# bonlime/sota_imagenet

Measured on AMD Instinct MI355X. Metric: images/sec (whole node) ResNet-50 bs=256/GPU @224px, higher is better.
Workload: dtype bf16; 1 GPU; ResNet-50 v1.5 train step (fwd+CE+bwd+allreduce+SGD), bs=256/GPU, 224px, configs[2] bf16 activations / fp32 accumulate+master; global_batch=256, image_size=224, parallelism=dp1

## Files before the change

### include/mi355rn.h

```cpp
#ifndef MI355RN_H
#define MI355RN_H

#include <stddef.h>
#include <stdint.h>

#ifdef __cplusplus
extern "C" {
#endif

typedef enum mi355_status {
  MI355_OK = 0,
  MI355_E_ARG = -1,
  MI355_E_HIP = -2,
  MI355_E_STATE = -3,
  MI355_E_NOMEM = -4
} mi355_status;

typedef enum mi355_dtype { MI355_F32 = 0, MI355_BF16 = 1, MI355_FP8 = 2 } mi355_dtype;

const char* mi355_last_error(void);
int mi355_version(void);
int mi355_device_count(void);


// ... 52 lines not shown
int mi355_stem_ingest(int dtype, const float* x_nchw, void* xpad, int N, int H, int W, void* stream);
int mi355_stem_fwd(int dtype, const void* xpad, const float* w_krsc, void* y, int N, int H, int W,
                   void* ws, size_t ws_bytes, void* stream);
int mi355_stem_wgrad(int dtype, const void* dy, const void* xpad, float* dw, float beta, int N, int H,
                     int W, void* ws, size_t ws_bytes, void* stream);
size_t mi355_stem_workspace_bytes(int dtype, int N, int H, int W);

size_t mi355_bn_workspace_bytes(int C);
int mi355_bn_fwd_train(int dtype, const void* x, const void* residual, void* out, const float* gamma,
                       const float* beta, float* running_mean, float* running_var, float* save_mean,
                       float* save_invstd, int M, int C, float eps, float momentum, int relu, void* ws,
                       size_t ws_bytes, void* stream);
int mi355_bn_fwd_train_partial(int dtype, const void* x, const void* residual, void* out, const float* gamma,
                               const float* beta, float* running_mean, float* running_var, float* save_mean,
                               float* save_invstd, int M, int C, float eps, float momentum, int relu, const float* partial,
                               int nblk, void* ws, size_t ws_bytes, void* stream);
int mi355_bn_fwd_eval(int dtype, const void* x, const void* residual, void* out, const float* gamma,
                      const float* beta, const float* running_mean, const float* running_var, int M,
                      int C, float eps, int relu, void* ws, size_t ws_bytes, void* stream);
int mi355_bn_bwd(int dtype, const void* dout, const void* out, const void* x, const float* gamma,
                 const float* save_mean, const float* save_invstd, void* dx, void* dz_out,
                 float* dgamma, float* dbeta, float beta_acc, int M, int C, int relu, void* ws,
                 size_t ws_bytes, void* stream);

int mi355_maxpool_fwd(int dtype, const void* x, void* y, uint8_t* idx, int N, int H, int W, int C,
                      void* stream);
int mi355_maxpool_bwd(int dtype, const void* dy, const uint8_t* idx, void* dx, int N, int H, int W,
                      int C, void* stream);

int mi355_gap_fwd(int dtype, const void* x, float* pooled, int N, int HW, int C, void* stream);
int mi355_gap_bwd(int dtype, const float* dpooled, void* dx, int N, int HW, int C, void* stream);

int mi355_ce_loss(const float* logits, const float* target, float smoothing, float grad_scale,
                  float* loss, float* row_loss, float* dlogits, int N, int C, void* stream);

int mi355_sgd_step(float* p, const float* g, float* m, size_t n, float lr, float momentum,
                   float weight_decay, float grad_scale, void* stream);
int mi355_sgd_step_ema(float* p, const float* g, float* m, float* ema, size_t n, float lr, float momentum,
                       float weight_decay, float grad_scale, float ema_decay, void* stream);

int mi355_adam_step(float* p, const float* g, float* m, float* v, size_t n, double beta1, double beta2, float eps,
                    float step_size, float bc2_sqrt, double lr, double weight_decay, int decoupled, float grad_scale,
                    void* stream);
int mi355_adam_step_ema(float* p, const float* g, float* m, float* v, float* ema, size_t n, double beta1, double beta2,
                        float eps, float step_size, float bc2_sqrt, double lr, double weight_decay, int decoupled,
                        float grad_scale, float ema_decay, void* stream);
// ... 164 lines not shown
```

### sota_imagenet_amd/csrc/bn.hip

```cpp
#include <hip/hip_fp8.h>

#include <algorithm>

#include "common.h"
#include "vec.h"

namespace mi355 {
namespace {

constexpr int MAXBLK = 512;

__device__ __forceinline__ void quant8(const float (&v)[8], float scale, uint8_t* dst, float& amax) {
  float c[8];
#pragma unroll
  for (int e = 0; e < 8; ++e) {
    const float r = (float)(bf16_t)v[e];
    amax = fmaxf(amax, fabsf(r));
    c[e] = __builtin_amdgcn_fmed3f(r * scale, 448.f, -448.f);
  }
  int lo = 0, hi = 0;
  lo = __builtin_amdgcn_cvt_pk_fp8_f32(c[0], c[1], lo, false);
  lo = __builtin_amdgcn_cvt_pk_fp8_f32(c[2], c[3], lo, true);
  hi = __builtin_amdgcn_cvt_pk_fp8_f32(c[4], c[5], hi, false);
  hi = __builtin_amdgcn_cvt_pk_fp8_f32(c[6], c[7], hi, true);
// ... 6 lines not shown
  if ((threadIdx.x & 63) == 0) wmax[threadIdx.x >> 6] = amax;
  __syncthreads();
  if (threadIdx.x == 0) {
    const float m = fmaxf(fmaxf(wmax[0], wmax[1]), fmaxf(wmax[2], wmax[3]));
    if (m > __uint_as_float(__atomic_load_n(dst, __ATOMIC_RELAXED))) atomicMax(dst, __float_as_uint(m));
  }
}

template <int V>
__device__ __forceinline__ void load_consts(const float* __restrict__ p, int c0, float (&v)[V]) {
#pragma unroll
  for (int q = 0; q < V / 4; ++q) {
    const f32x4 t = *reinterpret_cast<const f32x4*>(p + c0 + 4 * q);
    v[4 * q] = t[0]; v[4 * q + 1] = t[1]; v[4 * q + 2] = t[2]; v[4 * q + 3] = t[3];
  }
}

template <typename T, int V>
__device__ __forceinline__ void eca_grad(const EcaGrad& eg, int n, int C, int c0, float (&gv)[V]) {
  const float kn = eg.keep ? eg.keep[n] : 1.f;
  const size_t o = (size_t)n * C + c0;
#pragma unroll
  for (int e = 0; e < V; ++e) gv[e] = (float)(T)(gv[e] * kn * eg.gate[o + e] + eg.dpool[o + e]);
}

struct ReduceArgs {
  const void* x;
  const void* g;
  const void* mask;
  const uint8_t* bits;
  void* dz_out;
  const float* mean;
  const float* invstd;
  float* partial;
  float* pivot;
  int M, C;
  float slope;
  EcaGrad eg;
};

template <typename T, int MODE, int MASK, bool DZ>
__global__ __launch_bounds__(256) void bn_reduce_kernel(const ReduceArgs p) {
  constexpr int V = Vec16<T>::N;
  __shared__ __attribute__((aligned(16))) float red[2][256 * V];
  const int tpr_full = p.C / V;
  const int tpr = tpr_full < 256 ? tpr_full : 256;
// ... 47 lines not shown
#pragma unroll
        for (int e = 0; e < V; ++e) gv[e] = (b >> e) & 1u ? gv[e] : 0.f;
      } else if constexpr (MASK == 3) {
        const unsigned b = p.bits[off / V];
#pragma unroll
        for (int e = 0; e < V; ++e) gv[e] = (b >> e) & 1u ? gv[e] : gv[e] * p.slope;
      } else if constexpr (MASK == 1) {
        float mv[V];
        Vec16<T>::load(mk + off, mv);
#pragma unroll
        for (int e = 0; e < V; ++e) gv[e] = mv[e] > 0.f ? gv[e] : gv[e] * p.slope;
      } else if constexpr (MASK == 4) {
        eca_grad<T, V>(p.eg, m / p.eg.hw, p.C, c0, gv);
      }
      if constexpr (DZ) Vec16<T>::store(dz_out + off, gv);
#pragma unroll
      for (int e = 0; e < V; ++e) {
        const float xh = (xv[e] - mu[e]) * is[e];
        s1[e] += gv[e];
        s2[e] += gv[e] * xh;
      }
    }
  }
  int nrows, myrow;
  bool writer;
  if (tpr < 64) {
    for (int off = tpr; off < 64; off <<= 1) {
#pragma unroll
      for (int e = 0; e < V; ++e) {
        s1[e] += __shfl_xor(s1[e], off);
        s2[e] += __shfl_xor(s2[e], off);
      }
    }
    nrows = 4;
    myrow = tid >> 6;
    writer = (tid & 63) < tpr;
  } else {
    nrows = rpp;
    myrow = r;
    writer = true;
  }
  if (writer) {
#pragma unroll
    for (int e = 0; e < V; ++e) {
      red[0][(myrow * tpr + cv) * V + e] = s1[e];
      red[1][(myrow * tpr + cv) * V + e] = s2[e];
    }
  }
  __syncthreads();
  if (tid < tpr) {
#pragma unroll
    for (int e = 0; e < V; ++e) {
      float a = 0.f, b = 0.f;
      for (int rr = 0; rr < nrows; ++rr) {
        a += red[0][(rr * tpr + tid) * V + e];
        b += red[1][(rr * tpr + tid) * V + e];
      }
      const int c = (blockIdx.y * tpr + tid) * V + e;
      p.partial[((size_t)blockIdx.x * 2 + 0) * p.C + c] = a;
      p.partial[((size_t)blockIdx.x * 2 + 1) * p.C + c] = b;
    }
  }
}

struct FinalizeArgs {
  const float* partial;
  const float* pivot;
  int nblk, M, C;
  const float* gamma;
  const float* beta;
  float* running_mean;
  float* running_var;
  float* save_mean;
  float* save_invstd;
  float* scale;
  float* shift;
  float eps, momentum;
  const float* invstd;
  float* dgamma;
  float* dbeta;
  float beta_acc;
  float* coef;
};

static int fin_wide_mode() { return 2; }
// ... 151 lines not shown
#pragma unroll
      for (int e = 0; e < V; ++e) v[e] = v[e] > 0.f ? v[e] : (RELU == 2 ? 0.f : v[e] * p.slope);
    }
    if constexpr (!QONLY) Vec16<T>::store(out + i * V, v);
    if constexpr (Q) quant8(v, qs, p.qo.q + i * V, amax);
  }
  if constexpr (Q) amax_flush(amax, p.qo.amax);
}

struct BwdApplyArgs {
  const void* g;
  const void* mask;
  const uint8_t* bits;
  const void* x;
  const float* mean;
  const float* invstd;
  const float* coef;
  void* dx;
  size_t nvec;
  int cvecs, C;
  float slope;
  EcaGrad eg;
  QuantOut qo;
};

template <typename T, int MASK, bool Q = false, bool QONLY = false>
__global__ __launch_bounds__(256) void bn_bwd_apply_kernel(const BwdApplyArgs p) {
  constexpr int V = Vec16<T>::N;
  static_assert(!Q || V == 8, "the quantised twin exists for bf16 tensors");
  float qs = 1.f, amax = 0.f;
  if constexpr (Q) qs = p.qo.scale[0];
  const T* g = reinterpret_cast<const T*>(p.g);
  const T* mk = reinterpret_cast<const T*>(p.mask);
  const T* x = reinterpret_cast<const T*>(p.x);
  T* dx = reinterpret_cast<T*>(p.dx);
  const size_t stride = (size_t)gridDim.x * 256;
  size_t i = (size_t)blockIdx.x * 256 + threadIdx.x;
  const int c0 = (int)(i % p.cvecs) * V;
  float mu[V], is[V], k0[V], k1[V], k2[V];
  load_consts<V>(p.mean, c0, mu);
  load_consts<V>(p.invstd, c0, is);
  load_consts<V>(p.coef, c0, k0);
  load_consts<V>(p.coef + p.C, c0, k1);
  load_consts<V>(p.coef + 2 * p.C, c0, k2);
#pragma unroll 2
  for (; i < p.nvec; i += stride) {
    float gv[V], xv[V];
    Vec16<T>::load_nt(g + i * V, gv);
    Vec16<T>::load_nt(x + i * V, xv);
    if constexpr (MASK == 2) {
      const unsigned b = p.bits[i];
#pragma unroll
      for (int e = 0; e < V; ++e) gv[e] = (b >> e) & 1u ? gv[e] : 0.f;
    } else if constexpr (MASK == 3) {
      const unsigned b = p.bits[i];
#pragma unroll
      for (int e = 0; e < V; ++e) gv[e] = (b >> e) & 1u ? gv[e] : gv[e] * p.slope;
    } else if constexpr (MASK == 4) {
      eca_grad<T, V>(p.eg, (int)((i / p.cvecs) / (size_t)p.eg.hw), p.C, c0, gv);
    } else if constexpr (MASK == 1) {
      float mv[V];
      Vec16<T>::load(mk + i * V, mv);
#pragma unroll
      for (int e = 0; e < V; ++e) gv[e] = mv[e] > 0.f ? gv[e] : gv[e] * p.slope;
    }
#pragma unroll
    for (int e = 0; e < V; ++e) {
      const float xh = (xv[e] - mu[e]) * is[e];
      gv[e] = k0[e] * (gv[e] - k1[e] - xh * k2[e]);
    }
    if constexpr (!QONLY) Vec16<T>::store(dx + i * V, gv);
    if constexpr (Q) quant8(gv, qs, p.qo.q + i * V, amax);
  }
  if constexpr (Q) amax_flush(amax, p.qo.amax);
}

constexpr int SC = 64;

__device__ __forceinline__ __amdgpu_buffer_rsrc_t rsrc_of(const void* p, size_t bytes) {
  return __builtin_amdgcn_make_buffer_rsrc(const_cast<void*>(p), 0, (int)(bytes > 0xfffffffcull ? 0xfffffffcull : bytes), 0x00020000);
}
__device__ __forceinline__ uint4 buf16(__amdgpu_buffer_rsrc_t r, unsigned voff, unsigned soff, bool nt = false) {
  return nt ? __builtin_bit_cast(uint4, __builtin_amdgcn_raw_buffer_load_b128(r, voff, soff, 2))
            : __builtin_bit_cast(uint4, __builtin_amdgcn_raw_buffer_load_b128(r, voff, soff, 0));
}

template <typename T>
struct PoolGather {
  static constexpr int V = Vec16<T>::N;
  uint4 g[4];
  uint32_t id[4][V / 4];
  __device__ __forceinline__ void load(__amdgpu_buffer_rsrc_t rg, __amdgpu_buffer_rsrc_t ri, unsigned t, unsigned cv, int a, int b, int Ho, int Wo) {
    const unsigned go = (t * SC + cv * V) * (unsigned)sizeof(T), io = t * SC + cv * V;
#pragma unroll
    for (int w = 0; w < 4; ++w) {
      const bool ok = a + (w >> 1) < Ho && b + (w & 1) < Wo;
      const unsigned srow = (w >> 1) ? (unsigned)Wo * SC : 0u;
// ... 396 lines not shown

int launch_bn_bwd_finalize(const float* partial, int nblk, int M, int C, const float* gamma, const float* invstd,
                           float* dgamma, float* dbeta, float beta_acc, float* coef, hipStream_t s) {
  FinalizeArgs a{};
  a.partial = partial;
  a.nblk = nblk;
  a.M = M;
  a.C = C;
  a.gamma = gamma;
  a.invstd = invstd;
  a.dgamma = dgamma;
  a.dbeta = dbeta;
  a.beta_acc = beta_acc;
  a.coef = coef;
  if (fin_one_channel(C, nblk) && nblk > FIN_WIDE_ROWS) hipLaunchKernelGGL((bn_finalize_kernel<1, 1, 1024>), dim3(C), dim3(1024), 0, s, a);
  else if (fin_one_channel(C, nblk)) hipLaunchKernelGGL((bn_finalize_kernel<1, 1>), dim3(C), dim3(256), 0, s, a);
  else hipLaunchKernelGGL((bn_finalize_kernel<1, 4>), dim3(C / 4), dim3(256), 0, s, a);
  MI355_LAUNCH_CHECK();
  return 0;
}

int launch_bn_bwd_apply(int dtype, const void* g, const void* mask_src, const void* x, const float* mean,
                        const float* invstd, const float* coef, void* dx, int M, int C, hipStream_t s,
                        const uint8_t* relu_bits, float slope, QuantOut qo, const EcaGrad* eg) {
  MI355_TRY(check_c(dtype, C));
  const int V = 16 / (int)dtype_size(dtype);
  BwdApplyArgs a{};
  if (eg) a.eg = *eg;
  a.slope = slope;
  a.g = g;
  a.mask = mask_src;
  a.bits = relu_bits;
  a.x = x;
  a.mean = mean;
  a.invstd = invstd;
  a.coef = coef;
  a.dx = dx;
  a.nvec = (size_t)M * C / V;
  a.cvecs = C / V;
  a.C = C;
  const int blocks = elementwise_blocks(a.nvec, a.cvecs);
  const int mask = relu_bits ? (slope != 0.f ? 3 : 2) : mask_src ? 1 : 0;
  a.qo = qo;
  if (eg) {
    MI355_ARG(mask == 0 && !qo.q && eg->gate && eg->dpool && eg->hw > 0, "bn_bwd_apply: the ECA gradient source takes no mask / twin");
    if (dtype == MI355_F32) hipLaunchKernelGGL((bn_bwd_apply_kernel<float, 4>), dim3(blocks), dim3(256), 0, s, a);
    else hipLaunchKernelGGL((bn_bwd_apply_kernel<bf16_t, 4>), dim3(blocks), dim3(256), 0, s, a);
    MI355_LAUNCH_CHECK();
    return 0;
  }
  if (qo.q) {
    MI355_ARG(dtype == MI355_BF16 && mask != 1 && mask != 3 && qo.scale && qo.amax, "bn_bwd_apply: the e4m3 twin needs bf16 and a ReLU bit mask (or none)");
    if (mask == 2 && qo.only) hipLaunchKernelGGL((bn_bwd_apply_kernel<bf16_t, 2, true, true>), dim3(blocks), dim3(256), 0, s, a);
    else if (mask == 2) hipLaunchKernelGGL((bn_bwd_apply_kernel<bf16_t, 2, true>), dim3(blocks), dim3(256), 0, s, a);
    else if (qo.only) hipLaunchKernelGGL((bn_bwd_apply_kernel<bf16_t, 0, true, true>), dim3(blocks), dim3(256), 0, s, a);
    else hipLaunchKernelGGL((bn_bwd_apply_kernel<bf16_t, 0, true>), dim3(blocks), dim3(256), 0, s, a);
    MI355_LAUNCH_CHECK();
    return 0;
  }
#define MI355_BN_BWD_APPLY(TT)                                                                                  \
  switch (mask) {                                                                                               \
    case 0: hipLaunchKernelGGL((bn_bwd_apply_kernel<TT, 0>), dim3(blocks), dim3(256), 0, s, a); break;          \
    case 1: hipLaunchKernelGGL((bn_bwd_apply_kernel<TT, 1>), dim3(blocks), dim3(256), 0, s, a); break;          \
    case 2: hipLaunchKernelGGL((bn_bwd_apply_kernel<TT, 2>), dim3(blocks), dim3(256), 0, s, a); break;          \
    default: hipLaunchKernelGGL((bn_bwd_apply_kernel<TT, 3>), dim3(blocks), dim3(256), 0, s, a); break;         \
  }
// ... 55 lines not shown
```

### sota_imagenet_amd/csrc/common.h

```cpp
#pragma once
#include <hip/hip_runtime.h>
#include <cstdarg>
#include <cstdint>
#include <cstdio>
#include <cstring>

#include "../../include/mi355rn.h"

namespace mi355 {

typedef __bf16 bf16_t;

typedef float f32x4 __attribute__((ext_vector_type(4)));
typedef float f32x16 __attribute__((ext_vector_type(16)));
typedef __bf16 bf16x8 __attribute__((ext_vector_type(8)));
typedef __bf16 bf16x4 __attribute__((ext_vector_type(4)));
typedef short s16x4 __attribute__((ext_vector_type(4)));

void set_error(const char* fmt, ...);
int device_cus();
int probe_env(const char* name);

#define MI355_HIP(expr)                                                                         \
  do {                                                                                          \
// ... 181 lines not shown
                       float* scale, float* shift, float eps, float momentum, hipStream_t s);
int launch_bn_eval_coeffs(const float* gamma, const float* beta, const float* rm, const float* rv, float* scale,
                          float* shift, int C, float eps, hipStream_t s);
struct QuantOut {
  uint8_t* q = nullptr;
  const float* scale = nullptr;
  unsigned* amax = nullptr;
  bool only = false;
};
int launch_bn_apply(int dtype, const void* x, const float* scale, const float* shift, const void* residual,
                    const void* x2, const float* scale2, const float* shift2, void* out, int M, int C, int relu,
                    hipStream_t s, uint8_t* relu_bits = nullptr, QuantOut qo = QuantOut());
struct EcaGrad {
  const float* keep = nullptr;
  const float* gate = nullptr;
  const float* dpool = nullptr;
  int hw = 0;
};
int launch_bn_bwd_reduce(int dtype, const void* g, const void* mask_src, const void* x, const float* mean,
                         const float* invstd, void* dz_out, float* partial, int* nblk_out, int M, int C,
                         hipStream_t s, const uint8_t* relu_bits = nullptr, float slope = 0.f, const EcaGrad* eg = nullptr);
int launch_bn_bwd_finalize(const float* partial, int nblk, int M, int C, const float* gamma, const float* invstd,
                           float* dgamma, float* dbeta, float beta_acc, float* coef , hipStream_t s);
int launch_bn_bwd_apply(int dtype, const void* g, const void* mask_src, const void* x, const float* mean,
                        const float* invstd, const float* coef, void* dx, int M, int C, hipStream_t s,
                        const uint8_t* relu_bits = nullptr, float slope = 0.f, QuantOut qo = QuantOut(), const EcaGrad* eg = nullptr);
int launch_stem_bwd_reduce(int dtype, const void* dp, const uint8_t* idx, const uint8_t* bits, const void* y, const float* mean,
                           const float* invstd, float* partial, int* nblk_out, int N, int H, int W, int C, hipStream_t s);
int launch_stem_bwd_apply(int dtype, const void* dp, const uint8_t* idx, const uint8_t* bits, const void* y, const float* mean,
                          const float* invstd, const float* coef, void* dx, int N, int H, int W, int C, hipStream_t s);
int bn_max_blocks();
int launch_nchw_pad64(int dtype, const float* x_nchw, void* h_nhwc64, int N, int HW, hipStream_t s);
int launch_weight_pad_cast(int dtype, const float* w, void* wp, int Cout, int taps, int Cin, int Coutp, int Cinp, hipStream_t s);
int launch_nchw_im2col3s2(int dtype, const float* x, void* h, int N, int H, int W, hipStream_t s);
int launch_weight_unpad(const float* dwp, float* dw, float beta, int Cout, int taps, int Cin, int Cinp, hipStream_t s);
int launch_axpby(const float* src, float* dst, float beta, size_t n, hipStream_t s);
int launch_eca_residual_fwd(int dtype, const void* x, const float* w, int k, const float* keep, const void* shortcut, void* out, float* pooled, float* gate,
                            int N, int HW, int C, int act, hipStream_t s, const float* xs = nullptr, const float* xh = nullptr, const float* ss = nullptr,
                            const float* sh2 = nullptr, uint8_t* out_bits = nullptr, float* raw_ws = nullptr );
int launch_eca_residual_bwd(int dtype, const void* dout, const void* out, const void* x, const float* keep, const float* w, int k, const float* pooled,
                            const float* gate, void* dshortcut, void* dx, float* dw, float beta, float* ws, int N, int HW, int C, int act, hipStream_t s,
                            const float* xs = nullptr, const float* xh = nullptr, float* bn_row = nullptr, const float* bn_mean = nullptr,
                            const float* bn_invstd = nullptr, const uint8_t* out_bits = nullptr, const void* ds_y = nullptr, float* ds_row = nullptr,
                            const float* ds_mean = nullptr, const float* ds_invstd = nullptr);
int launch_fp8_scale_update(float* scale, unsigned* amax, int n, float headroom, hipStream_t s);

int launch_maxpool_fwd(int dtype, const void* x, void* y, uint8_t* idx, int N, int H, int W, int C, hipStream_t s);
int launch_bn_relu_maxpool(int dtype, const void* y, const float* scale, const float* shift, void* p, uint8_t* idx,
                           uint8_t* bits, int N, int H, int W, int C, hipStream_t s);
// ... 52 lines not shown
```

### sota_imagenet_amd/csrc/conv_api.cpp

```cpp
#include <algorithm>
#include <atomic>
#include <cstdio>
#include <cstdlib>
#include <mutex>
#include <set>
#include <string>

#include "conv_kernels.h"

namespace mi355 {

static thread_local std::string g_err;

void set_error(const char* fmt, ...) {
  char buf[1024];
  va_list ap;
  va_start(ap, fmt);
  vsnprintf(buf, sizeof(buf), fmt, ap);
  va_end(ap);
  g_err = buf;
}
const char* get_error() { return g_err.c_str(); }

int probe_env(const char* name) {
// ... 452 lines not shown
  MI355_ARG(ws && ws_bytes >= (size_t)2 * C * 4, "bn_eval: workspace too small");
  hipStream_t s = (hipStream_t)stream;
  float* scale = (float*)ws;
  float* shift = scale + C;
  MI355_TRY(launch_bn_eval_coeffs(gamma, beta, running_mean, running_var, scale, shift, C, eps, s));
  return launch_bn_apply(dtype, x, scale, shift, residual, nullptr, nullptr, nullptr, out, M, C, relu, s);
}

int mi355_bn_bwd(int dtype, const void* dout, const void* out, const void* x, const float* gamma,
                 const float* save_mean, const float* save_invstd, void* dx, void* dz_out, float* dgamma,
                 float* dbeta, float beta_acc, int M, int C, int relu, void* ws, size_t ws_bytes, void* stream) {
  MI355_ARG(ws && ws_bytes >= mi355_bn_workspace_bytes(C), "bn: workspace too small");
  hipStream_t s = (hipStream_t)stream;
  float* partial = (float*)ws;
  float* coef = partial + (size_t)bn_max_blocks() * 2 * C;
  int nblk = 0;
  const void* mask = relu ? out : nullptr;
  const float slope = relu == 2 ? 0.01f : 0.f;
  MI355_TRY(launch_bn_bwd_reduce(dtype, dout, mask, x, save_mean, save_invstd, dz_out, partial, &nblk, M, C, s, nullptr, slope));
  MI355_TRY(launch_bn_bwd_finalize(partial, nblk, M, C, gamma, save_invstd, dgamma, dbeta, beta_acc, coef, s));
  return launch_bn_bwd_apply(dtype, dout, mask, x, save_mean, save_invstd, coef, dx, M, C, s, nullptr, slope);
}

int mi355_maxpool_fwd(int dtype, const void* x, void* y, uint8_t* idx, int N, int H, int W, int C, void* stream) {
  return launch_maxpool_fwd(dtype, x, y, idx, N, H, W, C, (hipStream_t)stream);
}
int mi355_maxpool_bwd(int dtype, const void* dy, const uint8_t* idx, void* dx, int N, int H, int W, int C,
                      void* stream) {
  return launch_maxpool_bwd(dtype, dy, idx, dx, N, H, W, C, (hipStream_t)stream);
}
int mi355_gap_fwd(int dtype, const void* x, float* pooled, int N, int HW, int C, void* stream) {
  return launch_gap_fwd(dtype, x, pooled, N, HW, C, (hipStream_t)stream);
}
int mi355_gap_bwd(int dtype, const float* dpooled, void* dx, int N, int HW, int C, void* stream) {
  return launch_gap_bwd(dtype, dpooled, dx, N, HW, C, (hipStream_t)stream);
}
int mi355_ce_loss(const float* logits, const float* target, float smoothing, float grad_scale, float* loss,
                  float* row_loss, float* dlogits, int N, int C, void* stream) {
  return launch_ce(logits, target, smoothing, grad_scale, loss, row_loss, dlogits, N, C, (hipStream_t)stream);
}
int mi355_sgd_step(float* p, const float* g, float* m, size_t n, float lr, float momentum, float weight_decay,
                   float grad_scale, void* stream) {
  return launch_sgd(p, g, m, n, lr, momentum, weight_decay, grad_scale, (hipStream_t)stream);
}
int mi355_sgd_step_ema(float* p, const float* g, float* m, float* ema, size_t n, float lr, float momentum, float weight_decay,
                       float grad_scale, float ema_decay, void* stream) {
// ... 119 lines not shown
```

### sota_imagenet_amd/csrc/resnet_exec.cpp

```cpp
#include <cstdlib>
#include <string>
#include <vector>

#include "flat_model.h"

namespace mi355 {

namespace {

constexpr float BN_EPS = 1e-5f;
constexpr float FP8_HEADROOM = 2.f;
constexpr size_t PARAM_ALIGN = 64;
constexpr int MAX_EVENTS = 8192;

struct ConvBN {
  std::string conv_name, bn_name;
  int Cin, Cout, K, stride, pad;
  int Hin, Win, Hout, Wout;
  size_t w_off = 0, gamma_off = 0, beta_off = 0;
  size_t rm_off = 0, rv_off = 0;
  void* y = nullptr;
  void* w_cast = nullptr;
  void* w_tr = nullptr;
  float* stat = nullptr;
// ... 42 lines not shown
  uint8_t* a0_bits = nullptr;
  float *pooled = nullptr, *fc_tmp = nullptr, *dlogits_pad = nullptr, *dpooled = nullptr, *fc_wtr = nullptr;
  float *bn_partial = nullptr, *bn_coef = nullptr, *wg_partial = nullptr;
  float *bn_partial2 = nullptr, *bn_coef2 = nullptr;
  void* sk_ws[2] = {nullptr, nullptr};
  bool stream_k = true;
  bool fp8 = false;
  int q_n = 0;
  float* q_scale = nullptr;
  unsigned* q_amax = nullptr;
  void* gq[MAX_GSETS][4] = {};
  bool fp8_fwd_cal = false, fp8_bwd_cal = false;
  bool fp8_fwd_on = false, fp8_bwd_on = false;
  bool fp8_use_fwd = true, fp8_use_bwd = true;
  bool fp8_use_wgrad = true;
  bool fp8_keep_bf16 = false;
  bool fp8_lean = false;
  unsigned* sk_err_host = nullptr;
  PrepDesc* prep_table[2] = {nullptr, nullptr};
  int prep_layers = 0, prep_tiles = 0;
  void* gG[2] = {nullptr, nullptr};
  void* gsub = nullptr;
  bool ds_compact = true;
  void* gset[MAX_GSETS][4] = {};
  size_t max_c = 64;
  int nsets = 2;
  bool fuse_bn_bwd = false;
  bool fuse_bn_in = true;
  bool stem_fused_bwd = true;
  hipEvent_t w_done[MAX_GSETS] = {};
  hipEvent_t ds_done = nullptr;
  bool w_pending[MAX_GSETS] = {};
  int bwd_parity = 0;
  bool fwd_training_done = false;
  int next_seg = 0;
  void* cur_dout = nullptr;
  double fwd_flops = 0, train_flops = 0;

  unsigned prof_mask = 0;
  std::vector<hipEvent_t> ev;
  struct Rec {
    int cls;
    int tag;
    double flops, bytes;
  };
  std::vector<Rec> recs;
// ... 41 lines not shown
  hipStream_t stream;
  int idx = -1;
  Prof(mi355_ctx* ctx, int cls, double flops, double bytes, hipStream_t s, int tag = 0) : c(ctx), stream(s) {
    if (!(c->prof_mask & (1u << cls))) return;
    if ((c->recs.size() + 1) * 2 > c->ev.size()) return;
    idx = (int)c->recs.size();
    c->recs.push_back({cls, tag, flops, bytes});
    (void)hipEventRecord(c->ev[2 * idx], stream);
  }
  ~Prof() {
    if (idx >= 0) (void)hipEventRecord(c->ev[2 * idx + 1], stream);
  }
};

enum { PC_IGEMM128 = 0, PC_IGEMM64 = 1, PC_WGRAD128 = 2, PC_WGRAD64 = 3, PC_BN_REDUCE = 4, PC_BN_APPLY = 5, PC_OTHER = 6,
       PC_BN_BWD_APPLY = 7 };
inline int igemm_class(int ncols) { return ncols % 128 == 0 ? PC_IGEMM128 : PC_IGEMM64; }
inline int wgrad_class(int cout) { return cout % 128 == 0 ? PC_WGRAD128 : PC_WGRAD64; }

inline float* bn_partial_of(mi355_ctx* c, hipStream_t s) { return (c->wstream && s == c->wstream) ? c->bn_partial2 : c->bn_partial; }
inline void* sk_ws_of(mi355_ctx* c, hipStream_t s) {
  return c->stream_k ? c->sk_ws[(c->wstream && s == c->wstream) ? 1 : 0] : nullptr;
}
inline float* bn_coef_of(mi355_ctx* c, hipStream_t s) { return (c->wstream && s == c->wstream) ? c->bn_coef2 : c->bn_coef; }
double conv_flops(const mi355_ctx* c, const ConvBN& l) {
  return 2.0 * c->N * l.Hout * l.Wout * (double)l.Cout * l.Cin * l.K * l.K;
}

int conv_forward(mi355_ctx* c, ConvBN& l, const void* in, int training, float momentum, hipStream_t s, const ConvBN* bn_in = nullptr,
                 void* a_out = nullptr, uint8_t* a_bits = nullptr) {
  IgemmArgs a;
  build_fwd_args(a, c->N, l.Hin, l.Win, l.Cin, l.Cout, l.K, l.K, l.stride, l.pad);
  a.in = in;
  if (bn_in) {
    a.bn_in = bn_in->stat + 2 * bn_in->Cout;
    a.bn_in_a = a_out;
    a.bn_in_bits = a_bits;
  }
  a.stat_partial = training ? bn_partial_of(c, s) : nullptr;
  a.stat_rows_cap = (int)((size_t)bn_max_blocks() * c->max_c / l.Cout);
  a.sk_ws = sk_ws_of(c, s);
  a.wt = c->dtype == MI355_F32 ? (const void*)(c->params + l.w_off) : (const void*)l.w_cast;
  a.out = l.y;
  const double fl = conv_flops(c, l);
  const bool q = training && c->fp8_fwd_on && l.fp8_fwd;
  const double by = (double)c->N * l.Hin * l.Win * l.Cin * (q ? 1 : c->es) * (bn_in ? 2.0 + 1.0 / 16 : 1.0) + (double)c->N * l.Hout * l.Wout * l.Cout * c->es;
// ... 44 lines not shown

int bn_apply(mi355_ctx* c, ConvBN& l, const void* residual, ConvBN* l2, void* out, int relu, hipStream_t s,
             uint8_t* bits, uint8_t* q = nullptr, int qid = -1, bool q_only = false) {
  const int M = c->N * l.Hout * l.Wout, C = l.Cout;
  const int nin = 1 + (residual ? 1 : 0) + (l2 ? 1 : 0);
  QuantOut qo;
  if (q && bits && qid >= 0) {
    qo.q = q; qo.scale = c->q_scale + qid; qo.amax = c->q_amax + qid;
    qo.only = q_only && !residual && !l2;
  }
  Prof p(c, PC_BN_APPLY, 0, (double)M * C * (c->es * (nin + (qo.only ? 0 : 1)) + (qo.q ? 1 : 0)), s);
  return launch_bn_apply(c->dtype, l.y, l.stat + 2 * C, l.stat + 3 * C, residual, l2 ? l2->y : nullptr,
                         l2 ? l2->stat + 2 * C : nullptr, l2 ? l2->stat + 3 * C : nullptr, out, M, C, relu, s, bits, qo);
}

void* grad_twin(const mi355_ctx* c, const void* g) {
  for (int p = 0; p < c->nsets; ++p)
    for (int i = 0; i < 4; ++i)
      if (c->gset[p][i] == g) return c->gq[p][i];
  return nullptr;
}

int bn_backward(mi355_ctx* c, ConvBN& l, const void* g, const uint8_t* bits, void* dz_out, void* dx, float beta_acc,
                hipStream_t s) {
  const int M = c->N * l.Hout * l.Wout, C = l.Cout;
  int nblk = l.bwd_rows;
  l.bwd_rows = 0;
  const double mask_bytes = bits ? (double)M * C * c->es / 16 : 0.0;
  if (nblk == 0 || dz_out) {
    Prof p(c, PC_BN_REDUCE, 0, (double)M * C * c->es * (2 + (dz_out ? 1 : 0)) + mask_bytes, s);
    MI355_TRY(launch_bn_bwd_reduce(c->dtype, g, nullptr, l.y, l.stat, l.stat + C, dz_out, bn_partial_of(c, s), &nblk, M, C, s,
                                   bits, 0.f));
  }
  MI355_TRY(launch_bn_bwd_finalize(bn_partial_of(c, s), nblk, M, C, c->params + l.gamma_off, l.stat + C,
                                     c->grads + l.gamma_off, c->grads + l.beta_off, beta_acc, bn_coef_of(c, s), s));
  const uint8_t* bits2 = dz_out ? nullptr : bits;
  const void* g2 = dz_out ? dz_out : g;
  QuantOut qo;
  if (c->fp8 && l.qid_dy >= 0) {
    qo.q = (uint8_t*)grad_twin(c, dx); qo.scale = c->q_scale + l.qid_dy; qo.amax = c->q_amax + l.qid_dy;
    qo.only = c->fp8_lean && c->fp8_bwd_on && l.fp8_dgrad && l.fp8_wgrad && qo.q;
  }
  Prof p(c, PC_BN_BWD_APPLY, 0, (double)M * C * (c->es * (qo.only ? 2 : 3) + (qo.q ? 1 : 0)) + (bits2 ? mask_bytes : 0.0), s);
  return launch_bn_bwd_apply(c->dtype, g2, nullptr, l.y, l.stat, l.stat + C, bn_coef_of(c, s), dx, M, C, s, bits2, 0.f, qo);
}

int conv_wgrad(mi355_ctx* c, ConvBN& l, const void* dy, const void* x, float beta_acc, hipStream_t s) {
  WgradArgs a;
  build_wgrad_args(a, c->N, l.Hin, l.Win, l.Cin, l.Cout, l.K, l.K, l.stride, l.pad);
  a.dy = dy; a.x = x; a.partial = c->wg_partial;
  const size_t n = (size_t)l.Cout * l.K * l.K * l.Cin;
  void* dyq = c->fp8_bwd_on && l.fp8_wgrad ? grad_twin(c, dy) : nullptr;
  const double by = ((double)c->N * l.Hin * l.Win * l.Cin + (double)c->N * l.Hout * l.Wout * l.Cout) * (dyq ? 1 : c->es);
  if (dyq) {
    a.dy = dyq; a.x = l.in_q;
    {
      Prof p(c, wgrad_class(l.Cout), conv_flops(c, l), by, s, 2);
      MI355_TRY(launch_wgrad(MI355_FP8, a, l.splits8, s));
    }
    snprintf(l.k_wgrad, sizeof(l.k_wgrad), "%s", mi355_last_conv_kernel());
    return launch_splitk_reduce(c->wg_partial, l.splits8, n, c->grads + l.w_off, n, beta_acc, s, c->q_scale + l.qid_dy, c->q_scale + l.qid_in);
  }
  {
    Prof p(c, wgrad_class(l.Cout), conv_flops(c, l), by, s);
    MI355_TRY(launch_wgrad(c->dtype, a, l.splits, s));
  }
  snprintf(l.k_wgrad, sizeof(l.k_wgrad), "%s", mi355_last_conv_kernel());
// ... 238 lines not shown
  const int splits = plan_wgrad_splits(MI355_F32, N, P, 1, 2048);
  hipStream_t ws;
  MI355_TRY(c->fork(s, &ws));
  MI355_TRY(launch_wgrad(MI355_F32, w, splits, ws));
  MI355_TRY(launch_splitk_reduce(c->wg_partial, splits, (size_t)P * 2048, c->grads + c->fc_w_off, (size_t)O * 2048,
                                 beta_acc, ws));
  MI355_TRY(launch_fc(c->dlogits_pad, c->fc_wtr, c->dpooled, N, 2048, P, s));
  const Block& last = c->blocks.back();
  c->cur_dout = c->gG[0];
  c->bwd_parity = 0;
  return launch_gap_bwd(c->dtype, c->dpooled, c->cur_dout, N, last.Hout * last.Wout, last.Cout, s);
}

int backward_block(mi355_ctx* c, Block& b, Block* prev, float beta_acc, hipStream_t s) {
  void* G = c->cur_dout;
  void* Gn = G == c->gG[0] ? c->gG[1] : c->gG[0];
  const int par = c->bwd_parity;
  c->bwd_parity = (par + 1) % c->nsets;
  void** S = c->gset[par];
  void *B1 = S[0], *B2 = S[1], *B3 = S[2], *B4 = S[3];
  hipStream_t ws;
  const bool sub2 = sub2_ok(c, b, prev);
  MI355_TRY(acquire_set(c, par, s));
  MI355_TRY(bn_backward(c, b.c3, G, b.out_bits, nullptr, B1, beta_acc, s));
  MI355_TRY(c->fork(s, &ws));
  MI355_TRY(conv_wgrad(c, b.c3, B1, b.a2, beta_acc, ws));
  if (b.has_ds) {
    MI355_TRY(bn_backward(c, b.ds, G, b.out_bits, nullptr, B2, beta_acc, ws));
    if (sub2) MI355_TRY(conv_dgrad_compact(c, b.ds, B2, c->gsub, ws));
    else MI355_TRY(conv_dgrad(c, b.ds, B2, Gn, nullptr, ws));
    if (c->overlap) MI355_HIP(hipEventRecord(c->ds_done, ws));
    MI355_TRY(conv_wgrad(c, b.ds, B2, b.in, beta_acc, ws));
  }
  MI355_TRY(conv_dgrad(c, b.c3, B1, B3, nullptr, s, nullptr, &b.c2, b.a2_bits, beta_acc));
  MI355_TRY(bn_backward(c, b.c2, B3, b.a2_bits, nullptr, B3, beta_acc, s));
  MI355_TRY(c->fork(s, &ws));
  MI355_TRY(conv_wgrad(c, b.c2, B3, b.a1, beta_acc, ws));
  MI355_TRY(conv_dgrad(c, b.c2, B3, B4, nullptr, s, nullptr, &b.c1, b.a1_bits, beta_acc));
  MI355_TRY(bn_backward(c, b.c1, B4, b.a1_bits, nullptr, B4, beta_acc, s));
  MI355_TRY(c->fork(s, &ws));
  MI355_TRY(conv_wgrad(c, b.c1, B4, b.in, beta_acc, ws));
  if (b.has_ds) {
    if (c->overlap) MI355_HIP(hipStreamWaitEvent(s, c->ds_done, 0));
    MI355_TRY(conv_dgrad(c, b.c1, B4, Gn, sub2 ? c->gsub : Gn, s, nullptr, prev ? &prev->c3 : nullptr, prev ? prev->out_bits : nullptr, beta_acc, sub2));
    c->cur_dout = Gn;
  } else {
    MI355_TRY(conv_dgrad(c, b.c1, B4, G, G, s, b.out_bits, prev ? &prev->c3 : nullptr, prev ? prev->out_bits : nullptr, beta_acc));
// ... 109 lines not shown
  double f = conv_flops(c, c->stem), bw = 2 * conv_flops(c, c->stem) - conv_flops(c, c->stem);
  double tr = 2 * conv_flops(c, c->stem);
  (void)bw;
  for (auto& b : c->blocks) {
    const double fb = conv_flops(c, b.c1) + conv_flops(c, b.c2) + conv_flops(c, b.c3) + (b.has_ds ? conv_flops(c, b.ds) : 0);
    f += fb;
    tr += 3 * fb;
  }
  const double ffc = 2.0 * N * 2048 * num_classes;
  c->fwd_flops = f + ffc;
  c->train_flops = tr + 3 * ffc;

  const char* bad = nullptr;
  if (c->fp8) {
    plan_fp8(c, &bad);
    c->fp8_use_fwd = env_switch("MI355_FP8_FWD", 1, 1, &bad) != 0;
    c->fp8_use_bwd = env_switch("MI355_FP8_BWD", 1, 1, &bad) != 0;
  }
  c->stream_k = env_switch("MI355_STREAM_K", 1, 1, &bad) != 0;
  c->fuse_bn_bwd = env_switch("MI355_FUSE_BN_BWD", dtype == MI355_BF16 ? 1 : 0, 1, &bad) != 0;
  c->stem_fused_bwd = env_switch("MI355_STEM_FUSED", 1, 1, &bad) != 0;
  c->overlap = env_switch("MI355_WGRAD_STREAM", 1, 1, &bad) != 0;
  c->ds_compact = env_switch("MI355_DS_COMPACT", 1, 1, &bad) != 0;
  if (bad) {
    set_error("create: %s=%s is outside the switch's domain", bad, getenv(bad));
    mi355_resnet50_destroy(c);
    return MI355_E_ARG;
  }
  Arena ar;
  plan_arena(c, ar);
  c->arena_bytes = ar.size;
  if (device < 0) {
    *out = c;
    return 0;
  }
  hipError_t e = hipMalloc((void**)&c->arena, ar.size);
  if (e != hipSuccess) {
    set_error("create: hipMalloc(%zu bytes) -> %s", ar.size, hipGetErrorString(e));
    delete c;
    return MI355_E_NOMEM;
  }
  for (auto& sl : ar.slots) *sl.first = c->arena + sl.second;
  e = hipMemset(c->arena, 0, ar.size);
  if (e != hipSuccess) {
    set_error("create: hipMemset -> %s", hipGetErrorString(e));
    delete c;
// ... 398 lines not shown
```

### sota_imagenet_amd/ops.py

```python
import ctypes

import torch

from . import native
from .native import check, cur_stream, dtype_code, ptr


def _L():
    return native.lib()


def _need_cuda(*ts):
    for t in ts:
        if t is not None and not (t.is_cuda and t.is_contiguous()):
            raise ValueError("tensors must be contiguous CUDA (ROCm) tensors")


def _out_dim(h, k, s, p):
    return (h + 2 * p - k) // s + 1


def conv2d_fwd(x, w, stride=1, pad=0, stats=False):
    _need_cuda(x, w)
    N, H, W, Cin = x.shape
# ... 202 lines not shown
    C = x.shape[-1]
    M = x.numel() // C
    out = torch.empty_like(x)
    ws, n = _bn_ws(C, x.device)
    check(_L().mi355_bn_fwd_eval(dtype_code(x.dtype), ptr(x), ptr(residual), ptr(out), ptr(gamma), ptr(beta), ptr(running_mean),
                                 ptr(running_var), M, C, eps, int(relu), ptr(ws), n, cur_stream()))
    return out


def bn_bwd(dout, out, x, gamma, save_mean, save_invstd, relu=True, want_dz=False):
    _need_cuda(dout, out, x, gamma, save_mean, save_invstd)
    C = x.shape[-1]
    M = x.numel() // C
    dx = torch.empty_like(x)
    dz = torch.empty_like(x) if want_dz else None
    dg = torch.empty(C, dtype=torch.float32, device=x.device)
    db = torch.empty(C, dtype=torch.float32, device=x.device)
    ws, n = _bn_ws(C, x.device)
    check(_L().mi355_bn_bwd(dtype_code(x.dtype), ptr(dout), ptr(out), ptr(x), ptr(gamma), ptr(save_mean), ptr(save_invstd), ptr(dx),
                            ptr(dz), ptr(dg), ptr(db), 0.0, M, C, int(relu), ptr(ws), n, cur_stream()))
    return dx, dg, db, dz


def maxpool_fwd(x):
    _need_cuda(x)
    N, H, W, C = x.shape
    y = torch.empty((N, H // 2, W // 2, C), dtype=x.dtype, device=x.device)
    idx = torch.empty((N, H // 2, W // 2, C), dtype=torch.uint8, device=x.device)
    check(_L().mi355_maxpool_fwd(dtype_code(x.dtype), ptr(x), ptr(y), ptr(idx), N, H, W, C, cur_stream()))
    return y, idx


def maxpool_bwd(dy, idx, x_shape):
    _need_cuda(dy, idx)
    N, H, W, C = x_shape
    dx = torch.empty((N, H, W, C), dtype=dy.dtype, device=dy.device)
    check(_L().mi355_maxpool_bwd(dtype_code(dy.dtype), ptr(dy), ptr(idx), ptr(dx), N, H, W, C, cur_stream()))
    return dx


def gap_fwd(x):
    _need_cuda(x)
    N, H, W, C = x.shape
    pooled = torch.empty((N, C), dtype=torch.float32, device=x.device)
    check(_L().mi355_gap_fwd(dtype_code(x.dtype), ptr(x), ptr(pooled), N, H * W, C, cur_stream()))
    return pooled
# ... 401 lines not shown
```

Measured before the change: 14330 images/sec.

## Fuse downsample BN backward reduction into the block's final BN backward apply pass

In bottleneck blocks with a downsample branch, the c3 BN backward apply kernel now also reads the downsample BN's input and accumulates its per-channel gradient sums under the shared ReLU mask. It writes them as partial rows, which lets the downsample BN skip its own reduce pass over the gradient. The intent is to save one full read of the gradient and mask per downsample block. In exchange, the fused kernel loads an extra tensor, drops the loop unroll, and may launch fewer blocks because of the partial-row cap.

New measurement: 14510 images/sec (median of 6 runs). 1.01x the previous value.

```diff
diff --git a/include/mi355rn.h b/include/mi355rn.h
--- a/include/mi355rn.h
+++ b/include/mi355rn.h
@@ -98,6 +98,11 @@
                  const float* save_mean, const float* save_invstd, void* dx, void* dz_out,
                  float* dgamma, float* dbeta, float beta_acc, int M, int C, int relu, void* ws,
                  size_t ws_bytes, void* stream);
+
+int mi355_bn_bwd_sums2(int dtype, const void* dout, const uint8_t* bits, const void* x, const float* gamma, const float* save_mean,
+                       const float* save_invstd, const void* x2, const float* gamma2, const float* save_mean2, const float* save_invstd2,
+                       void* dx, void* dx2, float* dgamma, float* dbeta, float* dgamma2, float* dbeta2, int* rows2, int M, int C, void* ws,
+                       size_t ws_bytes, void* stream);
 
 int mi355_maxpool_fwd(int dtype, const void* x, void* y, uint8_t* idx, int N, int H, int W, int C,
                       void* stream);
diff --git a/sota_imagenet_amd/csrc/bn.hip b/sota_imagenet_amd/csrc/bn.hip
--- a/sota_imagenet_amd/csrc/bn.hip
+++ b/sota_imagenet_amd/csrc/bn.hip
@@ -52,6 +52,50 @@
   const size_t o = (size_t)n * C + c0;
 #pragma unroll
   for (int e = 0; e < V; ++e) gv[e] = (float)(T)(gv[e] * kn * eg.gate[o + e] + eg.dpool[o + e]);
+}
+
+template <int V>
+__device__ __forceinline__ void block_sums_to_row(float (&s1)[V], float (&s2)[V], float (&red)[2][256 * V], int tpr, float* __restrict__ row, int C) {
+  const int tid = threadIdx.x;
+  const int cv = tid % tpr, r = tid / tpr;
+  int nrows, myrow;
+  bool writer;
+  if (tpr < 64) {
+    for (int off = tpr; off < 64; off <<= 1) {
+#pragma unroll
+      for (int e = 0; e < V; ++e) {
+        s1[e] += __shfl_xor(s1[e], off);
+        s2[e] += __shfl_xor(s2[e], off);
+      }
+    }
+    nrows = 4;
+    myrow = tid >> 6;
+    writer = (tid & 63) < tpr;
+  } else {
+    nrows = 256 / tpr;
+    myrow = r;
+    writer = true;
+  }
+  if (writer) {
+#pragma unroll
+    for (int e = 0; e < V; ++e) {
+      red[0][(myrow * tpr + cv) * V + e] = s1[e];
+      red[1][(myrow * tpr + cv) * V + e] = s2[e];
+    }
+  }
+  __syncthreads();
+  if (tid < tpr) {
+#pragma unroll
+    for (int e = 0; e < V; ++e) {
+      float a = 0.f, b = 0.f;
+      for (int rr = 0; rr < nrows; ++rr) {
+        a += red[0][(rr * tpr + tid) * V + e];
+        b += red[1][(rr * tpr + tid) * V + e];
+      }
+      row[tid * V + e] = a;
+      row[C + tid * V + e] = b;
+    }
+  }
 }
 
 struct ReduceArgs {
@@ -145,45 +189,7 @@
       }
     }
   }
-  int nrows, myrow;
-  bool writer;
-  if (tpr < 64) {
-    for (int off = tpr; off < 64; off <<= 1) {
-#pragma unroll
-      for (int e = 0; e < V; ++e) {
-        s1[e] += __shfl_xor(s1[e], off);
-        s2[e] += __shfl_xor(s2[e], off);
-      }
-    }
-    nrows = 4;
-    myrow = tid >> 6;
-    writer = (tid & 63) < tpr;
-  } else {
-    nrows = rpp;
-    myrow = r;
-    writer = true;
-  }
-  if (writer) {
-#pragma unroll
-    for (int e = 0; e < V; ++e) {
-      red[0][(myrow * tpr + cv) * V + e] = s1[e];
-      red[1][(myrow * tpr + cv) * V + e] = s2[e];
-    }
-  }
-  __syncthreads();
-  if (tid < tpr) {
-#pragma unroll
-    for (int e = 0; e < V; ++e) {
-      float a = 0.f, b = 0.f;
-      for (int rr = 0; rr < nrows; ++rr) {
-        a += red[0][(rr * tpr + tid) * V + e];
-        b += red[1][(rr * tpr + tid) * V + e];
-      }
-      const int c = (blockIdx.y * tpr + tid) * V + e;
-      p.partial[((size_t)blockIdx.x * 2 + 0) * p.C + c] = a;
-      p.partial[((size_t)blockIdx.x * 2 + 1) * p.C + c] = b;
-    }
-  }
+  block_sums_to_row<V>(s1, s2, red, tpr, p.partial + (size_t)blockIdx.x * 2 * p.C + (size_t)blockIdx.y * tpr * V, p.C);
 }
 
 struct FinalizeArgs {
@@ -381,12 +387,17 @@
   float slope;
   EcaGrad eg;
   QuantOut qo;
+  const void* x2;
+  const float* mean2;
+  const float* invstd2;
+  float* partial2;
 };
 
-template <typename T, int MASK, bool Q = false, bool QONLY = false>
+template <typename T, int MASK, bool Q = false, bool QONLY = false, bool SUMS2 = false>
 __global__ __launch_bounds__(256) void bn_bwd_apply_kernel(const BwdApplyArgs p) {
   constexpr int V = Vec16<T>::N;
   static_assert(!Q || V == 8, "the quantised twin exists for bf16 tensors");
+  static_assert(!SUMS2 || MASK == 2, "the second BatchNorm's sums are taken under the ReLU bit mask");
   float qs = 1.f, amax = 0.f;
   if constexpr (Q) qs = p.qo.scale[0];
   const T* g = reinterpret_cast<const T*>(p.g);
@@ -402,11 +413,21 @@
   load_consts<V>(p.coef, c0, k0);
   load_consts<V>(p.coef + p.C, c0, k1);
   load_consts<V>(p.coef + 2 * p.C, c0, k2);
-#pragma unroll 2
+  const T* x2 = reinterpret_cast<const T*>(p.x2);
+  float mu2[SUMS2 ? V : 1], is2[SUMS2 ? V : 1], s1[SUMS2 ? V : 1], s2[SUMS2 ? V : 1];
+  if constexpr (SUMS2) {
+    load_consts<V>(p.mean2, c0, mu2);
+    load_consts<V>(p.invstd2, c0, is2);
+#pragma unroll
+    for (int e = 0; e < V; ++e) s1[e] = s2[e] = 0.f;
+  }
+  constexpr int UNROLL = SUMS2 ? 1 : 2;
+#pragma unroll UNROLL
   for (; i < p.nvec; i += stride) {
-    float gv[V], xv[V];
+    float gv[V], xv[V], x2v[SUMS2 ? V : 1];
     Vec16<T>::load_nt(g + i * V, gv);
     Vec16<T>::load_nt(x + i * V, xv);
+    if constexpr (SUMS2) Vec16<T>::load(x2 + i * V, x2v);
     if constexpr (MASK == 2) {
       const unsigned b = p.bits[i];
 #pragma unroll
@@ -423,6 +444,14 @@
 #pragma unroll
       for (int e = 0; e < V; ++e) gv[e] = mv[e] > 0.f ? gv[e] : gv[e] * p.slope;
     }
+    if constexpr (SUMS2) {
+#pragma unroll
+      for (int e = 0; e < V; ++e) {
+        const float xh2 = (x2v[e] - mu2[e]) * is2[e];
+        s1[e] += gv[e];
+        s2[e] += gv[e] * xh2;
+      }
+    }
 #pragma unroll
     for (int e = 0; e < V; ++e) {
       const float xh = (xv[e] - mu[e]) * is[e];
@@ -432,6 +461,12 @@
     if constexpr (Q) quant8(gv, qs, p.qo.q + i * V, amax);
   }
   if constexpr (Q) amax_flush(amax, p.qo.amax);
+  if constexpr (SUMS2) {
+    __shared__ __attribute__((aligned(16))) float red[2][256 * V];
+    const int tpr = p.cvecs < 256 ? p.cvecs : 256;
+    const int rpw = p.cvecs / tpr;
+    block_sums_to_row<V>(s1, s2, red, tpr, p.partial2 + (size_t)(blockIdx.x / rpw) * 2 * p.C + (size_t)(blockIdx.x % rpw) * tpr * V, p.C);
+  }
 }
 
 constexpr int SC = 64;
@@ -874,7 +909,7 @@
 
 int launch_bn_bwd_apply(int dtype, const void* g, const void* mask_src, const void* x, const float* mean,
                         const float* invstd, const float* coef, void* dx, int M, int C, hipStream_t s,
-                        const uint8_t* relu_bits, float slope, QuantOut qo, const EcaGrad* eg) {
+                        const uint8_t* relu_bits, float slope, QuantOut qo, const EcaGrad* eg, const BnSums2* sums2) {
   MI355_TRY(check_c(dtype, C));
   const int V = 16 / (int)dtype_size(dtype);
   BwdApplyArgs a{};
@@ -894,6 +929,24 @@
   const int blocks = elementwise_blocks(a.nvec, a.cvecs);
   const int mask = relu_bits ? (slope != 0.f ? 3 : 2) : mask_src ? 1 : 0;
   a.qo = qo;
+  if (sums2) {
+    MI355_ARG(mask == 2 && !eg && sums2->x2 && sums2->mean2 && sums2->invstd2 && sums2->partial && sums2->nblk,
+              "bn_bwd_apply: a second BatchNorm's sums need a ReLU bit mask and its tensor, statistics and row buffer");
+    MI355_ARG(!qo.q || (dtype == MI355_BF16 && qo.scale && qo.amax), "bn_bwd_apply: the e4m3 twin needs bf16 and a ReLU bit mask (or none)");
+    MI355_ARG(C == 256 || C == 512 || C == 1024 || C == 2048, "bn_bwd_apply: a second BatchNorm's sums cover C in {256, 512, 1024, 2048}, not %d", C);
+    const int rpw = a.cvecs > 256 ? a.cvecs / 256 : 1;
+    const int cap = (int)std::min<long long>((long long)sums2->rows_cap * rpw, 65536) / 4 * 4;
+    MI355_ARG(cap >= 4, "bn_bwd_apply: room for %d partial rows of the second BatchNorm", sums2->rows_cap);
+    const int blocks2 = std::min(blocks, cap);
+    a.x2 = sums2->x2; a.mean2 = sums2->mean2; a.invstd2 = sums2->invstd2; a.partial2 = sums2->partial;
+    *sums2->nblk = blocks2 / rpw;
+    if (qo.q && qo.only) hipLaunchKernelGGL((bn_bwd_apply_kernel<bf16_t, 2, true, true, true>), dim3(blocks2), dim3(256), 0, s, a);
+    else if (qo.q) hipLaunchKernelGGL((bn_bwd_apply_kernel<bf16_t, 2, true, false, true>), dim3(blocks2), dim3(256), 0, s, a);
+    else if (dtype == MI355_F32) hipLaunchKernelGGL((bn_bwd_apply_kernel<float, 2, false, false, true>), dim3(blocks2), dim3(256), 0, s, a);
+    else hipLaunchKernelGGL((bn_bwd_apply_kernel<bf16_t, 2, false, false, true>), dim3(blocks2), dim3(256), 0, s, a);
+    MI355_LAUNCH_CHECK();
+    return 0;
+  }
   if (eg) {
     MI355_ARG(mask == 0 && !qo.q && eg->gate && eg->dpool && eg->hw > 0, "bn_bwd_apply: the ECA gradient source takes no mask / twin");
     if (dtype == MI355_F32) hipLaunchKernelGGL((bn_bwd_apply_kernel<float, 4>), dim3(blocks), dim3(256), 0, s, a);
diff --git a/sota_imagenet_amd/csrc/common.h b/sota_imagenet_amd/csrc/common.h
--- a/sota_imagenet_amd/csrc/common.h
+++ b/sota_imagenet_amd/csrc/common.h
@@ -227,9 +227,18 @@
                          hipStream_t s, const uint8_t* relu_bits = nullptr, float slope = 0.f, const EcaGrad* eg = nullptr);
 int launch_bn_bwd_finalize(const float* partial, int nblk, int M, int C, const float* gamma, const float* invstd,
                            float* dgamma, float* dbeta, float beta_acc, float* coef , hipStream_t s);
+struct BnSums2 {
+  const void* x2 = nullptr;
+  const float* mean2 = nullptr;
+  const float* invstd2 = nullptr;
+  float* partial = nullptr;
+  int rows_cap = 0;
+  int* nblk = nullptr;
+};
 int launch_bn_bwd_apply(int dtype, const void* g, const void* mask_src, const void* x, const float* mean,
                         const float* invstd, const float* coef, void* dx, int M, int C, hipStream_t s,
-                        const uint8_t* relu_bits = nullptr, float slope = 0.f, QuantOut qo = QuantOut(), const EcaGrad* eg = nullptr);
+                        const uint8_t* relu_bits = nullptr, float slope = 0.f, QuantOut qo = QuantOut(), const EcaGrad* eg = nullptr,
+                        const BnSums2* sums2 = nullptr);
 int launch_stem_bwd_reduce(int dtype, const void* dp, const uint8_t* idx, const uint8_t* bits, const void* y, const float* mean,
                            const float* invstd, float* partial, int* nblk_out, int N, int H, int W, int C, hipStream_t s);
 int launch_stem_bwd_apply(int dtype, const void* dp, const uint8_t* idx, const uint8_t* bits, const void* y, const float* mean,
diff --git a/sota_imagenet_amd/csrc/conv_api.cpp b/sota_imagenet_amd/csrc/conv_api.cpp
--- a/sota_imagenet_amd/csrc/conv_api.cpp
+++ b/sota_imagenet_amd/csrc/conv_api.cpp
@@ -498,6 +498,26 @@
   return launch_bn_bwd_apply(dtype, dout, mask, x, save_mean, save_invstd, coef, dx, M, C, s, nullptr, slope);
 }
 
+int mi355_bn_bwd_sums2(int dtype, const void* dout, const uint8_t* bits, const void* x, const float* gamma, const float* save_mean,
+                       const float* save_invstd, const void* x2, const float* gamma2, const float* save_mean2, const float* save_invstd2, void* dx,
+                       void* dx2, float* dgamma, float* dbeta, float* dgamma2, float* dbeta2, int* rows2, int M, int C, void* ws, size_t ws_bytes,
+                       void* stream) {
+  MI355_ARG(ws && ws_bytes >= mi355_bn_workspace_bytes(C), "bn: workspace too small");
+  MI355_ARG(bits && rows2, "bn_bwd_sums2: the ReLU bit mask and the row count's address are required");
+  hipStream_t s = (hipStream_t)stream;
+  float* partial = (float*)ws;
+  float* coef = partial + (size_t)bn_max_blocks() * 2 * C;
+  float* coef2 = coef + 3 * (size_t)C;
+  int nblk = 0;
+  MI355_TRY(launch_bn_bwd_reduce(dtype, dout, nullptr, x, save_mean, save_invstd, nullptr, partial, &nblk, M, C, s, bits, 0.f));
+  MI355_TRY(launch_bn_bwd_finalize(partial, nblk, M, C, gamma, save_invstd, dgamma, dbeta, 0.f, coef, s));
+  BnSums2 s2;
+  s2.x2 = x2; s2.mean2 = save_mean2; s2.invstd2 = save_invstd2; s2.partial = partial; s2.rows_cap = bn_max_blocks(); s2.nblk = rows2;
+  MI355_TRY(launch_bn_bwd_apply(dtype, dout, nullptr, x, save_mean, save_invstd, coef, dx, M, C, s, bits, 0.f, QuantOut(), nullptr, &s2));
+  MI355_TRY(launch_bn_bwd_finalize(partial, *rows2, M, C, gamma2, save_invstd2, dgamma2, dbeta2, 0.f, coef2, s));
+  return launch_bn_bwd_apply(dtype, dout, nullptr, x2, save_mean2, save_invstd2, coef2, dx2, M, C, s, bits, 0.f);
+}
+
 int mi355_maxpool_fwd(int dtype, const void* x, void* y, uint8_t* idx, int N, int H, int W, int C, void* stream) {
   return launch_maxpool_fwd(dtype, x, y, idx, N, H, W, C, (hipStream_t)stream);
 }
diff --git a/sota_imagenet_amd/csrc/resnet_exec.cpp b/sota_imagenet_amd/csrc/resnet_exec.cpp
--- a/sota_imagenet_amd/csrc/resnet_exec.cpp
+++ b/sota_imagenet_amd/csrc/resnet_exec.cpp
@@ -88,6 +88,7 @@
   void* gG[2] = {nullptr, nullptr};
   void* gsub = nullptr;
   bool ds_compact = true;
+  bool ds_bn_sums = true;
   void* gset[MAX_GSETS][4] = {};
   size_t max_c = 64;
   int nsets = 2;
@@ -175,6 +176,7 @@
 inline void* sk_ws_of(mi355_ctx* c, hipStream_t s) {
   return c->stream_k ? c->sk_ws[(c->wstream && s == c->wstream) ? 1 : 0] : nullptr;
 }
+inline float* bn_partial_side(mi355_ctx* c, hipStream_t s) { return c->overlap && c->wstream ? c->bn_partial2 : bn_partial_of(c, s); }
 inline float* bn_coef_of(mi355_ctx* c, hipStream_t s) { return (c->wstream && s == c->wstream) ? c->bn_coef2 : c->bn_coef; }
 double conv_flops(const mi355_ctx* c, const ConvBN& l) {
   return 2.0 * c->N * l.Hout * l.Wout * (double)l.Cout * l.Cin * l.K * l.K;
@@ -265,7 +267,7 @@
 }
 
 int bn_backward(mi355_ctx* c, ConvBN& l, const void* g, const uint8_t* bits, void* dz_out, void* dx, float beta_acc,
-                hipStream_t s) {
+                hipStream_t s, ConvBN* l2 = nullptr) {
   const int M = c->N * l.Hout * l.Wout, C = l.Cout;
   int nblk = l.bwd_rows;
   l.bwd_rows = 0;
@@ -284,8 +286,16 @@
     qo.q = (uint8_t*)grad_twin(c, dx); qo.scale = c->q_scale + l.qid_dy; qo.amax = c->q_amax + l.qid_dy;
     qo.only = c->fp8_lean && c->fp8_bwd_on && l.fp8_dgrad && l.fp8_wgrad && qo.q;
   }
-  Prof p(c, PC_BN_BWD_APPLY, 0, (double)M * C * (c->es * (qo.only ? 2 : 3) + (qo.q ? 1 : 0)) + (bits2 ? mask_bytes : 0.0), s);
-  return launch_bn_bwd_apply(c->dtype, g2, nullptr, l.y, l.stat, l.stat + C, bn_coef_of(c, s), dx, M, C, s, bits2, 0.f, qo);
+  BnSums2 s2;
+  const bool sums2 = l2 && bits2 && c->ds_bn_sums;
+  if (sums2) {
+    s2.x2 = l2->y; s2.mean2 = l2->stat; s2.invstd2 = l2->stat + C;
+    s2.partial = bn_partial_side(c, s);
+    s2.rows_cap = std::min(bn_max_blocks(), (int)((size_t)bn_max_blocks() * c->max_c / C));
+    s2.nblk = &l2->bwd_rows;
+  }
+  Prof p(c, PC_BN_BWD_APPLY, 0, (double)M * C * (c->es * ((qo.only ? 2 : 3) + (sums2 ? 1 : 0)) + (qo.q ? 1 : 0)) + (bits2 ? mask_bytes : 0.0), s);
+  return launch_bn_bwd_apply(c->dtype, g2, nullptr, l.y, l.stat, l.stat + C, bn_coef_of(c, s), dx, M, C, s, bits2, 0.f, qo, nullptr, sums2 ? &s2 : nullptr);
 }
 
 int conv_wgrad(mi355_ctx* c, ConvBN& l, const void* dy, const void* x, float beta_acc, hipStream_t s) {
@@ -570,7 +580,7 @@
   hipStream_t ws;
   const bool sub2 = sub2_ok(c, b, prev);
   MI355_TRY(acquire_set(c, par, s));
-  MI355_TRY(bn_backward(c, b.c3, G, b.out_bits, nullptr, B1, beta_acc, s));
+  MI355_TRY(bn_backward(c, b.c3, G, b.out_bits, nullptr, B1, beta_acc, s, b.has_ds ? &b.ds : nullptr));
   MI355_TRY(c->fork(s, &ws));
   MI355_TRY(conv_wgrad(c, b.c3, B1, b.a2, beta_acc, ws));
   if (b.has_ds) {
@@ -726,6 +736,7 @@
   c->stem_fused_bwd = env_switch("MI355_STEM_FUSED", 1, 1, &bad) != 0;
   c->overlap = env_switch("MI355_WGRAD_STREAM", 1, 1, &bad) != 0;
   c->ds_compact = env_switch("MI355_DS_COMPACT", 1, 1, &bad) != 0;
+  c->ds_bn_sums = env_switch("MI355_DS_BN_SUMS", 1, 1, &bad) != 0;
   if (bad) {
     set_error("create: %s=%s is outside the switch's domain", bad, getenv(bad));
     mi355_resnet50_destroy(c);
diff --git a/sota_imagenet_amd/ops.py b/sota_imagenet_amd/ops.py
--- a/sota_imagenet_amd/ops.py
+++ b/sota_imagenet_amd/ops.py
@@ -248,6 +248,20 @@
     return dx, dg, db, dz
 
 
+def bn_bwd_sums2(dout, bits, x, gamma, save_mean, save_invstd, x2, gamma2, save_mean2, save_invstd2):
+    _need_cuda(dout, bits, x, gamma, save_mean, save_invstd, x2, gamma2, save_mean2, save_invstd2)
+    C = x.shape[-1]
+    M = x.numel() // C
+    dx, dx2 = torch.empty_like(x), torch.empty_like(x2)
+    dg, db, dg2, db2 = (torch.empty(C, dtype=torch.float32, device=x.device) for _ in range(4))
+    rows = ctypes.c_int(0)
+    ws, n = _bn_ws(C, x.device)
+    check(_L().mi355_bn_bwd_sums2(dtype_code(x.dtype), ptr(dout), ptr(bits), ptr(x), ptr(gamma), ptr(save_mean), ptr(save_invstd), ptr(x2), ptr(gamma2),
+                                  ptr(save_mean2), ptr(save_invstd2), ptr(dx), ptr(dx2), ptr(dg), ptr(db), ptr(dg2), ptr(db2), ctypes.byref(rows), M, C,
+                                  ptr(ws), n, cur_stream()))
+    return dx, dg, db, dx2, dg2, db2, rows.value
+
+
 def maxpool_fwd(x):
     _need_cuda(x)
     N, H, W, C = x.shape
```
